# lucidrains/progen

Measured on AMD Instinct MI355X. Metric: train tokens/sec (whole node), higher is better.
Workload: dtype bf16; 1 GPU; model=ProGen-1.2B, global_batch=64, seq_len=1024, parallelism=dp1

## Files before the change

### progen_amd/ops/hip/attention_bwd.hip

```cpp

#include "common.h"

#define DH 64
#define KT 64
#define ATTN_WAVES 4
#define ATTN_BLOCK (ATTN_WAVES * WAVE)
#define NEG_INF (-1e30f)

__device__ __forceinline__ int swz(int row, int byte_in_row) {
  return (byte_in_row ^ ((row & 7) << 4));
}

__device__ __forceinline__ void load_rope(const float* rsin,
                                          const float* rcos, long long pos,
                                          int d0, float* sv, float* cv) {
  *(f32x4*)(sv) = *(const f32x4*)(rsin + pos * DH + d0);
  *(f32x4*)(sv + 4) = *(const f32x4*)(rsin + pos * DH + d0 + 4);
  *(f32x4*)(cv) = *(const f32x4*)(rcos + pos * DH + d0);
  *(f32x4*)(cv + 4) = *(const f32x4*)(rcos + pos * DH + d0 + 4);
}

__device__ __forceinline__ int uk4(int k) { return ((k & 2) >> 1) | ((k & 8) >> 2); }

typedef __attribute__((__vector_size__(4 * sizeof(__bf16)))) __bf16 bf16x4t;
#define AS3 __attribute__((address_space(3)))

#define V5_WAVES 8
#define V5_BLOCK (V5_WAVES * WAVE)

__global__ __launch_bounds__(V5_BLOCK) void attn_bwd_kernel(
    const short* __restrict__ dout, const short* __restrict__ qkv,
    const short* __restrict__ halo,
    const short* __restrict__ out, const float* __restrict__ lse,
    float* __restrict__ dacc, float* __restrict__ dlook,
    float* __restrict__ dhalo,
    int B, int N, int H, int wsz) {
  const int window = blockIdx.x;
  const int head = blockIdx.y;
  const int batch = blockIdx.z;

  const int lane = threadIdx.x % WAVE;
  const int wid = threadIdx.x / WAVE;
  const int l15 = lane & 15;
  const int l4 = lane >> 4;
  const int pid = wid >> 1;
  const int phalf = wid & 1;

  const long long HD3 = 3LL * H * DH;
  const long long HD = (long long)H * DH;
  const long long HD2 = 2LL * H * DH;
  const long long qkv_bn = (long long)batch * N * HD3;
  const long long o_bn = (long long)batch * N * HD;
  const int q_off = head * DH;
  const int k_off = H * DH + head * DH;
  const int v_off = 2 * H * DH + head * DH;
  const long long look_bn = (long long)batch * N * HD2;
  const int lk_off = head * DH;
  const int lv_off = H * DH + head * DH;

  extern __shared__ __attribute__((aligned(16))) char smem[];
  char* k_lds = smem;
  char* kt_lds = smem + 8192;
  char* v_lds = smem + 16384;
  char* qt_base = smem + 24576;
  char* dot_base = qt_base + 4 * 8192;
  char* pds_base = dot_base + 4 * 8192;
  char* ds2_base = pds_base + 4 * 8192;
  float* d_base = (float*)(ds2_base + 4 * 8192);
  float* lse_base = (float*)(ds2_base + 4 * 8192 + 1024);

  char* qt_lds = qt_base + pid * 8192;
  char* dot_lds = dot_base + pid * 8192;
  char* pds_lds = pds_base + pid * 8192;
  char* ds2_lds = ds2_base + pid * 8192;
  float* d_lds = d_base + pid * 64;
  float* lse_lds = lse_base + pid * 64;

  const float scale = rsqrtf((float)DH);
  const int tiles = 2 * wsz / KT;
  const int chunks64 = wsz / 64;
  const int rounds = (chunks64 + 3) / 4;

  const int su_key = (int)threadIdx.x >> 3;
  const int su_d0 = ((int)threadIdx.x & 7) * 8;

  for (int round = 0; round < rounds; ++round) {
    const int c64 = round * 4 + pid;
    const bool active = c64 < chunks64;
    const int nactive = min(4, chunks64 - round * 4);
    const int chunk_off = c64 * 64 + phalf * 32;
    const int q0 = window * wsz + chunk_off;
    const int colbase = phalf * 32;

    bf16x8 qfrag[2][2];
    f32x4 dqacc[2][4];
#pragma unroll
    for (int m = 0; m < 2; ++m)
#pragma unroll
      for (int d = 0; d < 4; ++d) dqacc[m][d] = (f32x4){0.f, 0.f, 0.f, 0.f};

    if (active) {
#pragma unroll
      for (int m = 0; m < 2; ++m) {
        const int row = q0 + m * 16 + l15;
#pragma unroll
        for (int ks = 0; ks < 2; ++ks) {
          const int d0 = ks * 32 + 8 * l4;
          bf16x8 v = *(const bf16x8*)(qkv + qkv_bn + (long long)row * HD3 +
                                      q_off + d0);
          bf16x8 o;
#pragma unroll
          for (int j = 0; j < 8; ++j)
            ((short*)&o)[j] = f2bf(bf2f(((short*)&v)[j]) * scale);
          qfrag[m][ks] = o;
        }
      }
      {
        const int row = lane >> 1;
        const int col = colbase + row;
        const long long gq = qkv_bn + (long long)(q0 + row) * HD3 + q_off;
        const long long go = o_bn + (long long)(q0 + row) * HD + head * DH;
        float dsum = 0.f;
#pragma unroll
        for (int gg = 0; gg < 4; ++gg) {
          const int g = (lane & 1) * 4 + gg;
          const int d0 = g * 8;
          bf16x8 qv = *(const bf16x8*)(qkv + gq + d0);
          bf16x8 ov = *(const bf16x8*)(out + go + d0);
          bf16x8 dov = *(const bf16x8*)(dout + go + d0);
#pragma unroll
          for (int j = 0; j < 8; ++j) {
            const int d = d0 + j;
            *(short*)(qt_lds + d * 128 + swz(d, col * 2)) =
                f2bf(bf2f(((short*)&qv)[j]) * scale);
            *(short*)(dot_lds + d * 128 + swz(d, col * 2)) = ((short*)&dov)[j];
            dsum += bf2f(((short*)&ov)[j]) * bf2f(((short*)&dov)[j]);
          }
        }
        dsum += __shfl_xor(dsum, 1, 64);
        if ((lane & 1) == 0) {
          d_lds[col] = dsum;
          lse_lds[col] = lse[((long long)batch * H + head) * N + q0 + row];
        }
      }
    }
    __syncthreads();

    const int max_tile = active ? ((chunk_off + 31 + wsz) / KT) : -1;

    bf16x8 kreg, vreg;
    auto issue_loads = [&](int t) {
      const int kpos = (window - 1) * wsz + t * KT + su_key;
      if (kpos >= 0) {
        const long long base = qkv_bn + (long long)kpos * HD3;
        kreg = *(const bf16x8*)(qkv + base + k_off + su_d0);
        vreg = *(const bf16x8*)(qkv + base + v_off + su_d0);
      } else if (halo != nullptr) {
        const long long hb =
            ((long long)batch * wsz + (kpos + wsz)) * (2LL * H * DH);
        kreg = *(const bf16x8*)(halo + hb + head * DH + su_d0);
        vreg = *(const bf16x8*)(halo + hb + (long long)H * DH + head * DH +
                                su_d0);
      } else {
#pragma unroll
        for (int j = 0; j < 8; ++j) {
          ((short*)&kreg)[j] = 0;
          ((short*)&vreg)[j] = 0;
        }
      }
    };
    auto write_lds = [&]() {
      *(bf16x8*)(k_lds + su_key * 128 + swz(su_key, su_d0 * 2)) = kreg;
      *(bf16x8*)(v_lds + su_key * 128 + swz(su_key, su_d0 * 2)) = vreg;
#pragma unroll
      for (int j = 0; j < 8; ++j) {
        const int d = su_d0 + j;
        *(short*)(kt_lds + d * 128 + swz(d, su_key * 2)) =
            f2bf(bf2f(((short*)&kreg)[j]) * scale);
      }
    };

    issue_loads(0);
    write_lds();
    __syncthreads();

    for (int t = 0; t < tiles; ++t) {
      if (t + 1 < tiles) issue_loads(t + 1);
      const int kb = t * KT;
      const int c_min = max(0, (t * KT - wsz) / 64 - round * 4);
      const bool i_compute = active && t <= max_tile;

      if (i_compute) {
        f32x4 s[2][4];
#pragma unroll
        for (int m = 0; m < 2; ++m)
#pragma unroll
          for (int n = 0; n < 4; ++n) s[m][n] = (f32x4){0.f, 0.f, 0.f, 0.f};
        __builtin_amdgcn_s_setprio(1);
#pragma unroll
        for (int ks = 0; ks < 2; ++ks)
#pragma unroll
          for (int n = 0; n < 4; ++n) {
            const int key = n * 16 + l15;
            bf16x8 kf = *(const bf16x8*)(k_lds + key * 128 +
                                         swz(key, (ks * 32 + 8 * l4) * 2));
#pragma unroll
            for (int m = 0; m < 2; ++m)
              s[m][n] = __builtin_amdgcn_mfma_f32_16x16x32_bf16(
                  qfrag[m][ks], kf, s[m][n], 0, 0, 0);
          }
        __builtin_amdgcn_s_setprio(0);

#pragma unroll
        for (int m = 0; m < 2; ++m)
#pragma unroll
          for (int r = 0; r < 4; ++r) {
            const int rowiw = chunk_off + m * 16 + l4 * 4 + r;
            const float l = lse_lds[colbase + m * 16 + l4 * 4 + r];
#pragma unroll
            for (int n = 0; n < 4; ++n) {
              const int kpos_band = kb + n * 16 + l15;
              float v = ((float*)&s[m][n])[r];
              v = (kpos_band > rowiw + wsz) ? 0.f : __expf(v - l);
              ((float*)&s[m][n])[r] = v;
            }
          }
#pragma unroll
        for (int m = 0; m < 2; ++m)
#pragma unroll
          for (int n = 0; n < 4; ++n) {
            const int key = n * 16 + l15;
            const int row0 = colbase + m * 16 + l4 * 4;
            short pk[4];
#pragma unroll
            for (int r = 0; r < 4; ++r) pk[r] = f2bf(((float*)&s[m][n])[r]);
            *(unsigned long long*)(pds_lds + key * 128 + swz(key, row0 * 2)) =
                *(unsigned long long*)pk;
          }

        f32x4 dp[2][4];
#pragma unroll
        for (int m = 0; m < 2; ++m)
#pragma unroll
          for (int n = 0; n < 4; ++n) dp[m][n] = (f32x4){0.f, 0.f, 0.f, 0.f};
        __builtin_amdgcn_s_setprio(1);
#pragma unroll
        for (int ks = 0; ks < 2; ++ks)
#pragma unroll
          for (int m = 0; m < 2; ++m) {
            const int row = q0 + m * 16 + l15;
            const int d0 = ks * 32 + 8 * l4;
            bf16x8 dof = *(const bf16x8*)(dout + o_bn + (long long)row * HD +
                                          head * DH + d0);
#pragma unroll
            for (int n = 0; n < 4; ++n) {
              const int key = n * 16 + l15;
              bf16x8 vf = *(const bf16x8*)(v_lds + key * 128 + swz(key, d0 * 2));
              dp[m][n] = __builtin_amdgcn_mfma_f32_16x16x32_bf16(
                  dof, vf, dp[m][n], 0, 0, 0);
            }
          }
        __builtin_amdgcn_s_setprio(0);
#pragma unroll
        for (int m = 0; m < 2; ++m)
#pragma unroll
          for (int r = 0; r < 4; ++r) {
            const float dval = d_lds[colbase + m * 16 + l4 * 4 + r];
#pragma unroll
            for (int n = 0; n < 4; ++n) {
              float p = ((float*)&s[m][n])[r];
              float d = ((float*)&dp[m][n])[r];
              ((float*)&dp[m][n])[r] = p * (d - dval);
            }
          }
#pragma unroll
        for (int m = 0; m < 2; ++m)
#pragma unroll
          for (int n = 0; n < 4; ++n) {
            const int key = n * 16 + l15;
            const int row0 = colbase + m * 16 + l4 * 4;
            short dk4[4];
#pragma unroll
            for (int r = 0; r < 4; ++r) dk4[r] = f2bf(((float*)&dp[m][n])[r]);
            *(unsigned long long*)(ds2_lds + key * 128 +
                                   ((row0 * 2) ^ (uk4(key) * 32))) =
                *(unsigned long long*)dk4;
          }

        __builtin_amdgcn_s_setprio(1);
#pragma unroll
        for (int ks = 0; ks < 2; ++ks)
#pragma unroll
          for (int m = 0; m < 2; ++m) {
            const int krow1 = ks * 32 + l4 * 8 + (l15 >> 2);
            const int krow2 = krow1 + 4;
            const int colb = (colbase + m * 16 + (l15 & 3) * 4) * 2;
            auto p1 = (AS3 bf16x4t*)(ds2_lds + krow1 * 128 +
                                     (colb ^ (uk4(krow1) * 32)));
            auto p2 = (AS3 bf16x4t*)(ds2_lds + krow2 * 128 +
                                     (colb ^ (uk4(krow2) * 32)));
            bf16x4t f1 = __builtin_amdgcn_ds_read_tr16_b64_v4bf16(p1);
            bf16x4t f2 = __builtin_amdgcn_ds_read_tr16_b64_v4bf16(p2);
            bf16x8 dsf;
#pragma unroll
            for (int j = 0; j < 4; ++j) {
              ((__bf16*)&dsf)[j] = f1[j];
              ((__bf16*)&dsf)[j + 4] = f2[j];
            }
#pragma unroll
            for (int n = 0; n < 4; ++n) {
              const int d = n * 16 + l15;
              bf16x8 kf = *(const bf16x8*)(kt_lds + d * 128 +
                                           swz(d, (ks * 32 + 8 * l4) * 2));
              dqacc[m][n] = __builtin_amdgcn_mfma_f32_16x16x32_bf16(
                  dsf, kf, dqacc[m][n], 0, 0, 0);
            }
          }
        __builtin_amdgcn_s_setprio(0);
      }
      __syncthreads();

      if (t + 1 < tiles) write_lds();

      {
        const int dh0 = (wid >> 2) * 2;
        const int keyslot = (wid & 3) * 16 + l15;
        f32x4 dv[2], dk[2];
#pragma unroll
        for (int n = 0; n < 2; ++n) {
          dv[n] = (f32x4){0.f, 0.f, 0.f, 0.f};
          dk[n] = (f32x4){0.f, 0.f, 0.f, 0.f};
        }
        __builtin_amdgcn_s_setprio(1);
        for (int c = c_min; c < nactive; ++c) {
          char* pds_c = pds_base + c * 8192;
          char* ds2_c = ds2_base + c * 8192;
          char* dot_c = dot_base + c * 8192;
          char* qt_c = qt_base + c * 8192;
#pragma unroll
          for (int ks = 0; ks < 2; ++ks) {
            const int r0 = ks * 32 + 8 * l4;
            bf16x8 pf = *(const bf16x8*)(pds_c + keyslot * 128 +
                                         swz(keyslot, r0 * 2));
            bf16x8 dsf = *(const bf16x8*)(ds2_c + keyslot * 128 +
                                          ((r0 * 2) ^ (uk4(keyslot) * 32)));
#pragma unroll
            for (int n = 0; n < 2; ++n) {
              const int d = (dh0 + n) * 16 + l15;
              bf16x8 dof = *(const bf16x8*)(dot_c + d * 128 + swz(d, r0 * 2));
              bf16x8 qf = *(const bf16x8*)(qt_c + d * 128 + swz(d, r0 * 2));
              dv[n] = __builtin_amdgcn_mfma_f32_16x16x32_bf16(pf, dof, dv[n],
                                                              0, 0, 0);
              dk[n] = __builtin_amdgcn_mfma_f32_16x16x32_bf16(dsf, qf, dk[n],
                                                              0, 0, 0);
            }
          }
        }
        __builtin_amdgcn_s_setprio(0);
        const bool lookback = kb < wsz;
#pragma unroll
        for (int r = 0; r < 4; ++r) {
          const int kpos = (window - 1) * wsz + kb + (wid & 3) * 16 + l4 * 4 + r;
          float* dstv;
          float* dstk;
          if (kpos >= 0) {
            dstv = lookback
                ? dlook + look_bn + (long long)kpos * HD2 + lv_off
                : dacc + qkv_bn + (long long)kpos * HD3 + v_off;
            dstk = lookback
                ? dlook + look_bn + (long long)kpos * HD2 + lk_off
                : dacc + qkv_bn + (long long)kpos * HD3 + k_off;
          } else if (dhalo != nullptr) {
            const long long hb =
                ((long long)batch * wsz + (kpos + wsz)) * HD2;
            dstv = dhalo + hb + lv_off;
            dstk = dhalo + hb + lk_off;
          } else {
            continue;
          }
#pragma unroll
          for (int n = 0; n < 2; ++n) {
            const int dcol = (dh0 + n) * 16 + l15;
            float vv = ((float*)&dv[n])[r];
            float vk = ((float*)&dk[n])[r];
            if (round > 0) {
              vv += dstv[dcol];
              vk += dstk[dcol];
            }
            dstv[dcol] = vv;
            dstk[dcol] = vk;
          }
        }
      }
      __syncthreads();
    }

    if (active) {
#pragma unroll
      for (int m = 0; m < 2; ++m)
#pragma unroll
        for (int r = 0; r < 4; ++r) {
          const int row = q0 + m * 16 + l4 * 4 + r;
#pragma unroll
          for (int n = 0; n < 4; ++n)
            dacc[qkv_bn + (long long)row * HD3 + q_off + n * 16 + l15] =
                ((float*)&dqacc[m][n])[r];
        }
    }
    __syncthreads();
  }
}


__global__ __launch_bounds__(256) void attn_bwd_finalize_kernel(
    const float* __restrict__ dacc, const float* __restrict__ dlook,
    const float* __restrict__ rsin, const float* __restrict__ rcos,
    short* __restrict__ dqkv, int B, int N, int H, int wsz) {
  const long long HD3 = 3LL * H * DH;
  const long long HD2 = 2LL * H * DH;
  const int u = blockIdx.x * 256 + (int)threadIdx.x;
  if (u >= 3 * H * (DH / 8)) return;
  const int hslot = u >> 3;
  const int g = u & 7;
  const int d0 = g * 8;
  const long long BN = (long long)B * N;
  for (long long bn = blockIdx.y; bn < BN; bn += gridDim.y) {
    const int n = (int)(bn % N);

    const long long off = bn * HD3 + (long long)hslot * DH + d0;
    float x[8], sv[8], cv[8];
#pragma unroll
    for (int j = 0; j < 8; ++j) x[j] = dacc[off + j];
    if (hslot >= H && (n / wsz) < (N / wsz) - 1) {
      const long long loff = bn * HD2 + (long long)(hslot - H) * DH + d0;
#pragma unroll
      for (int j = 0; j < 8; ++j) x[j] += dlook[loff + j];
    }
    load_rope(rsin, rcos, n, d0, sv, cv);
#pragma unroll
    for (int p = 0; p < 4; ++p) {
      float y0 = x[2 * p], y1 = x[2 * p + 1];
      float s = sv[2 * p], c = cv[2 * p];
      x[2 * p] = y0 * c + y1 * s;
      x[2 * p + 1] = y1 * c - y0 * s;
    }
    bf16x8 o;
#pragma unroll
    for (int j = 0; j < 8; ++j) ((short*)&o)[j] = f2bf(x[j]);
    *(bf16x8*)(dqkv + off) = o;
  }
}

extern "C" {

hipError_t attn_bwd_launch(const void* dout, const void* qkv, const void* halo,
                           const float* rsin, const float* rcos,
                           const void* out, const float* lse, float* dacc,
                           float* dlook, float* dhalo, void* dqkv, int B, int N,
                           int H, int wsz, hipStream_t stream) {
  dim3 grid(N / wsz, H, B), block(V5_BLOCK);
  size_t lds = 24576 + 131072 + 2048;
  attn_bwd_kernel<<<grid, block, lds, stream>>>(
      (const short*)dout, (const short*)qkv, (const short*)halo,
      (const short*)out, lse, dacc, dlook, dhalo, B, N, H, wsz);
  hipError_t err = hipGetLastError();
  if (err != hipSuccess) return err;
  int gx = (3 * H * (DH / 8) + 255) / 256;
  long long bn_tot = (long long)B * N;
  int gy = (int)(bn_tot < 2048 ? bn_tot : 2048);
  dim3 fin_grid(gx, gy);
  attn_bwd_finalize_kernel<<<fin_grid, 256, 0, stream>>>(
      dacc, dlook, rsin, rcos, (short*)dqkv, B, N, H, wsz);
  return hipGetLastError();
}

}
```

### progen_amd/ops/hip/bindings.cpp

```cpp

#include <torch/extension.h>

#include "checks.h"
#include "kernels.h"

using namespace chk;


static std::vector<at::Tensor> ln_shift_fwd_impl(const char* op,
                                                 const at::Tensor& x,
                                                 const at::Tensor* res,
                                                 const at::Tensor& g,
                                                 bool shift, double eps) {
  const bool bf = dtype_bf16_or_fp32(op, ARG(x));
  dtype_same(op, ARG(g), ARG(x));
  if (res) dtype_same(op, Arg{"res", *res}, ARG(x));
  contiguous_rank(op, ARG(x), 3);
  const int64_t B = x.size(0), N = x.size(1), D = x.size(2);
  if (res) contiguous_shape(op, Arg{"res", *res}, x.sizes());
  contiguous_numel(op, ARG(g), D);
  multiple_of(op, "D", D, 16);
  const int Di = extent_int(op, "D", D), Ni = extent_int(op, "N", N);
  const int R = extent_int(op, "B*N", B * N);
  same_gpu(op, {ARG(x), ARG(g)});
// ... 34 lines not shown
  dtype_same(op, ARG(dy), xa);
  dtype_same(op, ARG(g), xa);
  if (ds) dtype_same(op, Arg{"ds", *ds}, xa);
  dtype_is(op, ARG(mean), at::kFloat);
  dtype_is(op, ARG(rstd), at::kFloat);
  contiguous_rank(op, xa, 3);
  const int64_t B = x.size(0), N = x.size(1), D = x.size(2);
  contiguous_shape(op, ARG(dy), x.sizes());
  if (ds) contiguous_shape(op, Arg{"ds", *ds}, x.sizes());
  contiguous_numel(op, ARG(g), D);
  contiguous_numel(op, ARG(mean), B * N);
  contiguous_numel(op, ARG(rstd), B * N);
  multiple_of(op, "D", D, 16);
  const int Di = extent_int(op, "D", D), Ni = extent_int(op, "N", N);
  const int R = extent_int(op, "B*N", B * N);
  same_gpu(op, {xa, ARG(dy), ARG(g), ARG(mean), ARG(rstd)});
  if (ds) same_gpu(op, {xa, Arg{"ds", *ds}});

  DeviceScope dev(x);
  const int nblocks = std::min(R, 1024);
  auto dx = at::empty_like(x);
  auto dw_part = at::empty({nblocks, D}, x.options().dtype(at::kFloat));
  LAUNCH(op, ln_shift_bwd_launch(
                 dy.data_ptr(), ds ? ds->data_ptr() : nullptr, x.data_ptr(),
                 g.data_ptr(), mean.data_ptr<float>(), rstd.data_ptr<float>(),
                 dx.data_ptr(), dw_part.data_ptr<float>(), nblocks, R, Ni, Di,
                 shift, bf, dev.stream));
  auto dw = dw_part.sum(0).to(x.scalar_type());
  return {dx, dw};
}

std::vector<at::Tensor> ln_shift_bwd(const at::Tensor& dy, const at::Tensor& x,
                                     const at::Tensor& g,
                                     const at::Tensor& mean,
                                     const at::Tensor& rstd, bool shift) {
  return ln_shift_bwd_impl("ln_shift_bwd", dy, c10::nullopt, ARG(x), g, mean,
                           rstd, shift);
}

std::vector<at::Tensor> ln_shift_res_bwd(const at::Tensor& dy,
                                         const c10::optional<at::Tensor>& ds,
                                         const at::Tensor& s_in,
                                         const at::Tensor& g,
                                         const at::Tensor& mean,
                                         const at::Tensor& rstd, bool shift) {
  return ln_shift_bwd_impl("ln_shift_res_bwd", dy, ds, ARG(s_in), g, mean,
                           rstd, shift);
}


at::Tensor glu_fwd(const at::Tensor& h) {
  const char* op = "glu_fwd";
  const bool bf = dtype_bf16_or_fp32(op, ARG(h));
  CHK(h.dim() >= 1, op, "h", h.dim(), "must have at least 1 dim");
  contiguous(op, ARG(h));
  const int64_t H2 = h.size(-1), rows = leading_rows(h);
  multiple_of(op, "H2", H2, 16);
  const int H = extent_int(op, "H2", H2) / 2;
  extent(op, "rows", rows, INT64_MAX);
  same_gpu(op, {ARG(h)});

  DeviceScope dev(h);
  auto sizes = h.sizes().vec();
  sizes.back() = H;
  auto y = at::empty(sizes, h.options());
  LAUNCH(op, glu_fwd_launch(h.data_ptr(), y.data_ptr(), rows, H, bf,
                            dev.stream));
  return y;
}

at::Tensor glu_bwd(const at::Tensor& dy, const at::Tensor& h) {
  const char* op = "glu_bwd";
  const bool bf = dtype_bf16_or_fp32(op, ARG(h));
  dtype_same(op, ARG(dy), ARG(h));
  CHK(h.dim() >= 1, op, "h", h.dim(), "must have at least 1 dim");
  contiguous(op, ARG(h));
  const int64_t H2 = h.size(-1), rows = leading_rows(h);
  auto dy_sizes = h.sizes().vec();
  dy_sizes.back() = H2 / 2;
  contiguous_shape(op, ARG(dy), dy_sizes);
  multiple_of(op, "H2", H2, 16);
  const int H = extent_int(op, "H2", H2) / 2;
  extent(op, "rows", rows, INT64_MAX);
  same_gpu(op, {ARG(h), ARG(dy)});

  DeviceScope dev(h);
  auto dh = at::empty_like(h);
  LAUNCH(op, glu_bwd_launch(dy.data_ptr(), h.data_ptr(), dh.data_ptr(), rows,
                            H, bf, dev.stream));
  return dh;
}

at::Tensor gelu_fwd(const at::Tensor& h) {
  const char* op = "gelu_fwd";
  const bool bf = dtype_bf16_or_fp32(op, ARG(h));
  contiguous(op, ARG(h));
  multiple_of(op, "h.numel()", h.numel(), 8);
  extent(op, "h.numel()", h.numel(), INT64_MAX);
  same_gpu(op, {ARG(h)});

  DeviceScope dev(h);
  auto y = at::empty_like(h);
  LAUNCH(op, gelu_fwd_launch(h.data_ptr(), y.data_ptr(), h.numel(), bf,
                             dev.stream));
  return y;
}

at::Tensor gelu_bwd(const at::Tensor& dy, const at::Tensor& h) {
  const char* op = "gelu_bwd";
  const bool bf = dtype_bf16_or_fp32(op, ARG(h));
  dtype_same(op, ARG(dy), ARG(h));
  contiguous(op, ARG(h));
  contiguous_shape(op, ARG(dy), h.sizes());
  multiple_of(op, "h.numel()", h.numel(), 8);
  extent(op, "h.numel()", h.numel(), INT64_MAX);
  same_gpu(op, {ARG(h), ARG(dy)});

  DeviceScope dev(h);
  auto dh = at::empty_like(h);
  LAUNCH(op, gelu_bwd_launch(dy.data_ptr(), h.data_ptr(), dh.data_ptr(),
                             h.numel(), bf, dev.stream));
  return dh;
}


static constexpr int64_t kCeMaxRows = 4 * (int64_t)INT_MAX;

std::vector<at::Tensor> ce_fwd(const at::Tensor& logits,
                               const at::Tensor& targets) {
  const char* op = "ce_fwd";
  const bool bf = dtype_bf16_or_fp32(op, ARG(logits));
  dtype_is(op, ARG(targets), at::kLong);
  CHK(logits.dim() >= 1, op, "logits", logits.dim(),
      "must have at least 1 dim");
  contiguous(op, ARG(logits));
  const int64_t R = leading_rows(logits);
  contiguous_numel(op, ARG(targets), R);
  const int V = extent_int(op, "V", logits.size(-1));
  extent(op, "rows", R, kCeMaxRows);
  same_gpu(op, {ARG(logits), ARG(targets)});

  DeviceScope dev(logits);
  auto nll = at::empty(targets.sizes(), logits.options().dtype(at::kFloat));
  auto lse = at::empty_like(nll);
  LAUNCH(op, ce_fwd_launch(logits.data_ptr(),
                           (const long long*)targets.data_ptr<int64_t>(),
                           nll.data_ptr<float>(), lse.data_ptr<float>(), R, V,
                           bf, dev.stream));
  return {nll, lse};
}

at::Tensor ce_bwd(const at::Tensor& dnll, const at::Tensor& logits,
                  const at::Tensor& targets, const at::Tensor& lse) {
  const char* op = "ce_bwd";
  const bool bf = dtype_bf16_or_fp32(op, ARG(logits));
  dtype_is(op, ARG(targets), at::kLong);
  dtype_is(op, ARG(dnll), at::kFloat);
  dtype_is(op, ARG(lse), at::kFloat);
  CHK(logits.dim() >= 1, op, "logits", logits.dim(),
      "must have at least 1 dim");
  contiguous(op, ARG(logits));
  const int64_t R = leading_rows(logits);
  contiguous_numel(op, ARG(targets), R);
  contiguous_numel(op, ARG(dnll), R);
  contiguous_numel(op, ARG(lse), R);
  const int V = extent_int(op, "V", logits.size(-1));
  extent(op, "rows", R, kCeMaxRows);
  same_gpu(op, {ARG(logits), ARG(targets), ARG(dnll), ARG(lse)});

  DeviceScope dev(logits);
  auto dlogits = at::empty_like(logits);
  LAUNCH(op, ce_bwd_launch(dnll.data_ptr<float>(), logits.data_ptr(),
                           (const long long*)targets.data_ptr<int64_t>(),
                           lse.data_ptr<float>(), dlogits.data_ptr(), R, V, bf,
                           dev.stream));
  return dlogits;
}


at::Tensor grad_sumsq(const at::Tensor& grads) {
  const char* op = "grad_sumsq";
  const bool bf = dtype_bf16_or_fp32(op, ARG(grads));
  contiguous(op, ARG(grads));
  multiple_of(op, "grads.numel()", grads.numel(), bf ? 8 : 4);
  extent(op, "grads.numel()", grads.numel(), INT64_MAX);
  same_gpu(op, {ARG(grads)});

  DeviceScope dev(grads);
  auto out = at::zeros({1}, grads.options().dtype(at::kFloat));
  LAUNCH(op, grad_sumsq_launch(grads.data_ptr(), out.data_ptr<float>(),
                               grads.numel(), bf, dev.stream));
  return out;
}

void fused_adamw(at::Tensor& master, at::Tensor& params,
                 const at::Tensor& grads, at::Tensor& exp_avg,
                 at::Tensor& exp_avg_sq, const at::Tensor& chunk_starts,
                 const at::Tensor& chunk_ends, const at::Tensor& chunk_decay,
                 double lr, double b1, double b2, double eps, double wd,
                 at::Tensor& step_dev, double grad_scale,
                 const at::Tensor& clip_coef, int64_t shard_off) {
  const char* op = "fused_adamw";
  const bool bf = dtype_bf16_or_fp32(op, ARG(params));
  dtype_same(op, ARG(grads), ARG(params));
  dtype_is(op, ARG(master), at::kFloat);
  dtype_is(op, ARG(exp_avg), at::kFloat);
  dtype_is(op, ARG(exp_avg_sq), at::kFloat);
  dtype_is(op, ARG(chunk_starts), at::kLong);
  dtype_is(op, ARG(chunk_ends), at::kLong);
  dtype_is(op, ARG(chunk_decay), at::kInt);
  dtype_is(op, ARG(step_dev), at::kInt);
  dtype_is(op, ARG(clip_coef), at::kFloat);
  contiguous(op, ARG(params));
  contiguous(op, ARG(master));
  contiguous(op, ARG(chunk_starts));
  contiguous_numel(op, ARG(grads), params.numel());
  contiguous_numel(op, ARG(exp_avg), master.numel());
  contiguous_numel(op, ARG(exp_avg_sq), master.numel());
  contiguous_numel(op, ARG(chunk_ends), chunk_starts.numel());
  contiguous_numel(op, ARG(chunk_decay), chunk_starts.numel());
  contiguous_numel(op, ARG(step_dev), 1);
  contiguous_numel(op, ARG(clip_coef), 1);
  CHK(shard_off >= 0, op, "shard_off", shard_off, "must be >= 0");
  CHK(shard_off <= params.numel() - master.numel(), op,
      "shard_off + master.numel()", shard_off + master.numel(),
      "must be <= params.numel() = ", params.numel());
  const int nchunks = extent_int(op, "nchunks", chunk_starts.numel());
  same_gpu(op, {ARG(params), ARG(grads), ARG(master), ARG(exp_avg),
                ARG(exp_avg_sq), ARG(chunk_starts), ARG(chunk_ends),
                ARG(chunk_decay), ARG(step_dev), ARG(clip_coef)});

  DeviceScope dev(params);
  LAUNCH(op, fused_adamw_launch(
                 master.data_ptr<float>(), params.data_ptr(), grads.data_ptr(),
                 exp_avg.data_ptr<float>(), exp_avg_sq.data_ptr<float>(),
                 (const long long*)chunk_starts.data_ptr<int64_t>(),
                 (const long long*)chunk_ends.data_ptr<int64_t>(),
                 chunk_decay.data_ptr<int>(), nchunks, (float)lr, (float)b1,
                 (float)b2, (float)eps, (float)wd, step_dev.data_ptr<int>(),
                 (float)grad_scale, clip_coef.data_ptr<float>(), bf,
                 (long long)shard_off, dev.stream));
}


at::Tensor rope_qkv(const at::Tensor& qkv, const at::Tensor& rsin,
                    const at::Tensor& rcos) {
  const char* op = "rope_qkv";
  dtype_is(op, ARG(qkv), at::kBFloat16);
  dtype_is(op, ARG(rsin), at::kFloat);
  dtype_is(op, ARG(rcos), at::kFloat);
  contiguous_rank(op, ARG(qkv), 3);
  const int64_t B = qkv.size(0), N = qkv.size(1), C = qkv.size(2);
  rope_table(op, ARG(rsin), N);
  rope_table(op, ARG(rcos), N);
  multiple_of(op, "qkv.size(2)", C, 3 * 64);
  const int Bi = extent_int(op, "B", B), Ni = extent_int(op, "N", N);
  const int H = extent_int(op, "heads", C / (3 * 64));
  same_gpu(op, {ARG(qkv), ARG(rsin), ARG(rcos)});

  DeviceScope dev(qkv);
  auto qkv_rot = at::empty_like(qkv);
  LAUNCH(op, rope_qkv_launch(qkv.data_ptr(), rsin.data_ptr<float>(),
                             rcos.data_ptr<float>(), qkv_rot.data_ptr(), Bi,
                             Ni, H, dev.stream));
  return qkv_rot;
}

std::vector<at::Tensor> attn_fwd(const at::Tensor& qkv_rot, int64_t heads,
                                 int64_t window,
                                 const c10::optional<at::Tensor>& halo) {
  const char* op = "attn_fwd";
  const int H = extent_int(op, "heads", heads, kGridYZ);
  const int wsz = extent_int(op, "window", window);
  dtype_is(op, ARG(qkv_rot), at::kBFloat16);
  if (halo) dtype_same(op, Arg{"halo", *halo}, ARG(qkv_rot));
  contiguous_rank(op, ARG(qkv_rot), 3);
  const int64_t B = qkv_rot.size(0), N = qkv_rot.size(1);
  CHK(qkv_rot.size(2) == 3 * heads * 64, op, "qkv_rot.size(2)",
      qkv_rot.size(2), "must be 3*heads*64 = ", 3 * heads * 64);
  if (halo)
    contiguous_shape(op, Arg{"halo", *halo}, {B, window, 2 * heads * 64});
  multiple_of(op, "window", window, 64);
  multiple_of(op, "N", N, window);
  const int Bi = extent_int(op, "B", B, kGridYZ);
  const int Ni = extent_int(op, "N", N);
  same_gpu(op, {ARG(qkv_rot)});
  if (halo) same_gpu(op, {ARG(qkv_rot), Arg{"halo", *halo}});

  DeviceScope dev(qkv_rot);
  auto out = at::empty({B, N, heads * 64}, qkv_rot.options());
  auto lse = at::empty({B, heads, N}, qkv_rot.options().dtype(at::kFloat));
  LAUNCH(op, attn_fwd_launch(qkv_rot.data_ptr(),
                             halo ? halo->data_ptr() : nullptr, out.data_ptr(),
                             lse.data_ptr<float>(), Bi, Ni, H, wsz,
                             dev.stream));
  return {out, lse};
}

std::vector<at::Tensor> attn_bwd(const at::Tensor& dout, const at::Tensor& qkv,
                                 const at::Tensor& rsin,
                                 const at::Tensor& rcos, const at::Tensor& out,
                                 const at::Tensor& lse, int64_t heads,
                                 int64_t window,
                                 const c10::optional<at::Tensor>& halo) {
  const char* op = "attn_bwd";
  const int H = extent_int(op, "heads", heads, kGridYZ);
  const int wsz = extent_int(op, "window", window);
  dtype_is(op, ARG(qkv), at::kBFloat16);
  dtype_same(op, ARG(dout), ARG(qkv));
  dtype_same(op, ARG(out), ARG(qkv));
  if (halo) dtype_same(op, Arg{"halo", *halo}, ARG(qkv));
  dtype_is(op, ARG(lse), at::kFloat);
  dtype_is(op, ARG(rsin), at::kFloat);
  dtype_is(op, ARG(rcos), at::kFloat);
  contiguous_rank(op, ARG(qkv), 3);
  const int64_t B = qkv.size(0), N = qkv.size(1);
  CHK(qkv.size(2) == 3 * heads * 64, op, "qkv.size(2)", qkv.size(2),
      "must be 3*heads*64 = ", 3 * heads * 64);
  contiguous_shape(op, ARG(out), {B, N, heads * 64});
  contiguous_shape(op, ARG(dout), {B, N, heads * 64});
  contiguous_shape(op, ARG(lse), {B, heads, N});
  rope_table(op, ARG(rsin), N);
  rope_table(op, ARG(rcos), N);
  if (halo)
    contiguous_shape(op, Arg{"halo", *halo}, {B, window, 2 * heads * 64});
  multiple_of(op, "window", window, 64);
  multiple_of(op, "N", N, window);
  const int Bi = extent_int(op, "B", B, kGridYZ);
  const int Ni = extent_int(op, "N", N);
  same_gpu(op, {ARG(qkv), ARG(dout), ARG(out), ARG(lse), ARG(rsin),
                ARG(rcos)});
  if (halo) same_gpu(op, {ARG(qkv), Arg{"halo", *halo}});

  DeviceScope dev(qkv);
  const auto f32 = qkv.options().dtype(at::kFloat);
  auto dacc = at::empty_like(qkv, f32);
  auto dlook = at::empty({B, N, 2 * heads * 64}, f32);
  auto dqkv = at::empty_like(qkv);
  auto dhalo = halo ? at::empty({B, window, 2 * heads * 64}, f32)
                    : at::Tensor();
  LAUNCH(op, attn_bwd_launch(
                 dout.data_ptr(), qkv.data_ptr(),
                 halo ? halo->data_ptr() : nullptr, rsin.data_ptr<float>(),
                 rcos.data_ptr<float>(), out.data_ptr(), lse.data_ptr<float>(),
                 dacc.data_ptr<float>(), dlook.data_ptr<float>(),
                 halo ? dhalo.data_ptr<float>() : nullptr, dqkv.data_ptr(), Bi,
                 Ni, H, wsz, dev.stream));
  if (halo) return {dqkv, dhalo};
  return {dqkv};
}


std::vector<at::Tensor> sgu_fwd(const at::Tensor& xa, const at::Tensor& g_ln,
                                const at::Tensor& w, const at::Tensor& bias) {
  const char* op = "sgu_fwd";
  dtype_is(op, ARG(xa), at::kBFloat16);
  dtype_same(op, ARG(g_ln), ARG(xa));
  dtype_same(op, ARG(w), ARG(xa));
  contiguous_rank(op, ARG(xa), 3);
  const int64_t B = xa.size(0), N = xa.size(1), D = xa.size(2);
  contiguous_shape(op, ARG(g_ln), xa.sizes());
  contiguous_shape(op, ARG(w), {N, N});
  CHK(bias.numel() == N, op, "bias", bias.numel(), "must have ", N,
      " elements");
  multiple_of(op, "N", N, 256);
  multiple_of(op, "D", D, 64);
  const int Bi = extent_int(op, "B", B, kGridYZ);
  const int Ni = extent_int(op, "N", N);
  const int Di = extent_int(op, "D", D, 64 * kGridYZ);
  same_gpu(op, {ARG(xa), ARG(g_ln), ARG(w), ARG(bias)});

  DeviceScope dev(xa);
  auto bias_f = bias.to(at::kFloat).contiguous().view({-1});
  auto out = at::empty_like(xa);
  auto gate_out = at::empty_like(xa);
  LAUNCH(op, sgu_fwd_launch(xa.data_ptr(), g_ln.data_ptr(), w.data_ptr(),
                            bias_f.data_ptr<float>(), out.data_ptr(),
                            gate_out.data_ptr(), Bi, Ni, Di, dev.stream));
  return {out, gate_out};
}

at::Tensor sgu_dgate(const at::Tensor& t_in, const at::Tensor& w) {
  const char* op = "sgu_dgate";
  dtype_is(op, ARG(t_in), at::kBFloat16);
  dtype_same(op, ARG(w), ARG(t_in));
  contiguous_rank(op, ARG(t_in), 3);
  const int64_t B = t_in.size(0), N = t_in.size(1), D = t_in.size(2);
  contiguous_shape(op, ARG(w), {N, N});
  multiple_of(op, "N", N, 256);
  multiple_of(op, "D", D, 64);
  const int Bi = extent_int(op, "B", B, kGridYZ);
  const int Ni = extent_int(op, "N", N);
  const int Di = extent_int(op, "D", D, 64 * kGridYZ);
  same_gpu(op, {ARG(t_in), ARG(w)});

  DeviceScope dev(t_in);
  auto dg = at::empty_like(t_in);
  LAUNCH(op, sgu_dgate_launch(t_in.data_ptr(), w.data_ptr(), dg.data_ptr(),
                              Bi, Ni, Di, dev.stream));
  return dg;
}

at::Tensor sgu_dw(const at::Tensor& t_in, const at::Tensor& g_ln,
                  const at::Tensor& tri_m, const at::Tensor& tri_k) {
  const char* op = "sgu_dw";
  dtype_is(op, ARG(t_in), at::kBFloat16);
  dtype_same(op, ARG(g_ln), ARG(t_in));
  dtype_is(op, ARG(tri_m), at::kInt);
  dtype_is(op, ARG(tri_k), at::kInt);
  contiguous_rank(op, ARG(t_in), 3);
  const int64_t B = t_in.size(0), N = t_in.size(1), D = t_in.size(2);
  contiguous_shape(op, ARG(g_ln), t_in.sizes());
  contiguous(op, ARG(tri_m));
  contiguous_numel(op, ARG(tri_k), tri_m.numel());
  multiple_of(op, "N", N, 64);
  multiple_of(op, "D", D, 32);
  const int ntri = extent_int(op, "tri_m.numel()", tri_m.numel());
  const int Bi = extent_int(op, "B", B, kGridYZ);
  const int Ni = extent_int(op, "N", N);
  const int Di = extent_int(op, "D", D, 768 * kGridYZ);
  same_gpu(op, {ARG(t_in), ARG(g_ln), ARG(tri_m), ARG(tri_k)});

  DeviceScope dev(t_in);
  auto dw = at::zeros({N, N}, t_in.options().dtype(at::kFloat));
  LAUNCH(op, sgu_dw_launch(t_in.data_ptr(), g_ln.data_ptr(),
                           dw.data_ptr<float>(), tri_m.data_ptr<int>(),
                           tri_k.data_ptr<int>(), ntri, Bi, Ni, Di,
                           dev.stream));
  return dw;
}


static const uint32_t* crc32c_tables() {
  static uint32_t tbl[8][256];
  static bool init = false;
  if (!init) {
    for (int i = 0; i < 256; ++i) {
      uint32_t c = (uint32_t)i;
      for (int k = 0; k < 8; ++k) c = (c >> 1) ^ ((c & 1) ? 0x82F63B78u : 0);
      tbl[0][i] = c;
    }
    for (int t = 1; t < 8; ++t)
      for (int i = 0; i < 256; ++i)
        tbl[t][i] = (tbl[t - 1][i] >> 8) ^ tbl[0][tbl[t - 1][i] & 0xFF];
    init = true;
  }
  return &tbl[0][0];
}

uint32_t crc32c_host(py::bytes data) {
  const uint32_t* T = crc32c_tables();
  char* buf;
  Py_ssize_t len;
  if (PyBytes_AsStringAndSize(data.ptr(), &buf, &len) != 0)
    throw std::runtime_error("crc32c: expected bytes");
  const uint8_t* p = (const uint8_t*)buf;
  uint32_t c = 0xFFFFFFFFu;
  size_t n = (size_t)len;
  while (n >= 8) {
    uint32_t lo, hi;
    memcpy(&lo, p, 4);
    memcpy(&hi, p + 4, 4);
    lo ^= c;
    c = T[7 * 256 + (lo & 0xFF)] ^ T[6 * 256 + ((lo >> 8) & 0xFF)] ^
        T[5 * 256 + ((lo >> 16) & 0xFF)] ^ T[4 * 256 + (lo >> 24)] ^
        T[3 * 256 + (hi & 0xFF)] ^ T[2 * 256 + ((hi >> 8) & 0xFF)] ^
        T[1 * 256 + ((hi >> 16) & 0xFF)] ^ T[0 * 256 + (hi >> 24)];
    p += 8;
    n -= 8;
  }
  while (n--) c = T[(c ^ *p++) & 0xFF] ^ (c >> 8);
  return c ^ 0xFFFFFFFFu;
}

at::Tensor colsum(const at::Tensor& dy) {
  const char* op = "colsum";
  dtype_is(op, ARG(dy), at::kBFloat16);
  contiguous_rank(op, ARG(dy), 2);
  multiple_of(op, "C", dy.size(1), 8);
  extent(op, "R", dy.size(0), INT_MAX);
  const int C = extent_int(op, "C", dy.size(1));
  same_gpu(op, {ARG(dy)});

  DeviceScope dev(dy);
  auto out = at::zeros({dy.size(1)}, dy.options().dtype(at::kFloat));
  LAUNCH(op, colsum_launch(dy.data_ptr(), out.data_ptr<float>(), dy.size(0),
                           C, dev.stream));
  return out;
}

at::Tensor fp8_quantize(const at::Tensor& t, const at::Tensor& scale) {
  const char* op = "fp8_quantize";
  dtype_is(op, ARG(t), at::kBFloat16);
  dtype_is(op, ARG(scale), at::kFloat);
  contiguous(op, ARG(t));
  contiguous_numel(op, ARG(scale), 1);
  multiple_of(op, "t.numel()", t.numel(), 8);
  extent(op, "t.numel()", t.numel(), INT64_MAX);
  same_gpu(op, {ARG(t), ARG(scale)});

  DeviceScope dev(t);
  auto out = at::empty_like(t, t.options().dtype(at::kFloat8_e4m3fn));
  LAUNCH(op, quant_e4m3_launch(t.data_ptr(), out.data_ptr(),
                               scale.data_ptr<float>(), t.numel(),
                               dev.stream));
  return out;
}

at::Tensor fp8_quantize_t(const at::Tensor& w, const at::Tensor& scale) {
  const char* op = "fp8_quantize_t";
  dtype_is(op, ARG(w), at::kBFloat16);
  dtype_is(op, ARG(scale), at::kFloat);
  contiguous_rank(op, ARG(w), 2);
  contiguous_numel(op, ARG(scale), 1);
  multiple_of(op, "rows", w.size(0), 2);
  const int Nr = extent_int(op, "rows", w.size(0));
  const int Kc = extent_int(op, "cols", w.size(1));
  extent(op, "tiles", ((w.size(0) + 63) / 64) * ((w.size(1) + 63) / 64),
         INT_MAX);
  same_gpu(op, {ARG(w), ARG(scale)});

  DeviceScope dev(w);
  auto out = at::empty({w.size(1), w.size(0)},
                       w.options().dtype(at::kFloat8_e4m3fn));
  LAUNCH(op, quant_e4m3_t_launch(w.data_ptr(), out.data_ptr(),
                                 scale.data_ptr<float>(), Nr, Kc, dev.stream));
  return out;
}

PYBIND11_MODULE(TORCH_EXTENSION_NAME, m) {
  m.def("sgu_fwd", &sgu_fwd, "SGU causal spatial matmul forward");
  m.def("sgu_dgate", &sgu_dgate, "SGU backward: dgate");
  m.def("sgu_dw", &sgu_dw, "SGU backward: dW");
  m.def("ln_shift_fwd", &ln_shift_fwd, "fused LN+shift forward");
  m.def("ln_shift_bwd", &ln_shift_bwd, "fused LN+shift backward");
  m.def("ln_shift_res_fwd", &ln_shift_res_fwd,
        "residual-add-fused LN+shift forward");
  m.def("ln_shift_res_bwd", &ln_shift_res_bwd,
        "residual-add-fused LN+shift backward");
  m.def("glu_fwd", &glu_fwd, "GLU-GELU forward");
  m.def("glu_bwd", &glu_bwd, "GLU-GELU backward");
  m.def("gelu_fwd", &gelu_fwd, "GELU forward");
  m.def("gelu_bwd", &gelu_bwd, "GELU backward");
  m.def("ce_fwd", &ce_fwd, "fused CE forward (nll, lse)");
  m.def("ce_bwd", &ce_bwd, "fused CE backward");
  m.def("grad_sumsq", &grad_sumsq, "sum of squares of flat grads");
  m.def("fused_adamw", &fused_adamw, "fused clip+AdamW over flat space",
        py::arg("master"), py::arg("params"), py::arg("grads"),
        py::arg("exp_avg"), py::arg("exp_avg_sq"), py::arg("chunk_starts"),
        py::arg("chunk_ends"), py::arg("chunk_decay"), py::arg("lr"),
        py::arg("b1"), py::arg("b2"), py::arg("eps"), py::arg("wd"),
        py::arg("step_dev"), py::arg("grad_scale"), py::arg("clip_coef"),
        py::arg("shard_off") = 0);
  m.def("rope_qkv", &rope_qkv, "pre-rotation of qkv (rotary on q,k,v)");
  m.def("attn_fwd", &attn_fwd, "fused local attention forward",
        py::arg("qkv_rot"), py::arg("heads"), py::arg("window"),
        py::arg("halo") = py::none());
  m.def("attn_bwd", &attn_bwd, "fused local attention backward",
        py::arg("dout"), py::arg("qkv"), py::arg("rsin"), py::arg("rcos"),
        py::arg("out"), py::arg("lse"), py::arg("heads"), py::arg("window"),
        py::arg("halo") = py::none());
  m.def("crc32c", &crc32c_host, "CRC-32C (slicing-by-8, host)");
  m.def("colsum", &colsum, "bf16 column sum (bias grads), fp32 accum");
  m.def("fp8_quantize", &fp8_quantize, "fused bf16 -> e4m3 at device scale");
  m.def("fp8_quantize_t", &fp8_quantize_t,
        "fused transpose-quantize (N,K) bf16 -> (K,N) e4m3");
}
```

### progen_amd/ops/hip/kernels.h

```cpp
#pragma once
#include <hip/hip_runtime.h>

extern "C" {

hipError_t ln_shift_fwd_launch(const void* x, const void* res, const void* g,
                               void* y, void* s_out, float* mean, float* rstd,
                               int R, int N, int D, float eps, bool shift,
                               bool is_bf16, hipStream_t stream);
hipError_t ln_shift_bwd_launch(const void* dy, const void* ds, const void* x,
                               const void* g, const float* mean,
                               const float* rstd, void* dx, float* dw_part,
                               int nblocks, int R, int N, int D, bool shift,
                               bool is_bf16, hipStream_t stream);

hipError_t glu_fwd_launch(const void* h, void* y, long long rows, int H,
                          bool is_bf16, hipStream_t stream);
hipError_t glu_bwd_launch(const void* dy, const void* h, void* dh,
                          long long rows, int H, bool is_bf16,
                          hipStream_t stream);
hipError_t gelu_fwd_launch(const void* h, void* y, long long total_elems,
                           bool is_bf16, hipStream_t stream);
hipError_t gelu_bwd_launch(const void* dy, const void* h, void* dh,
                           long long total_elems, bool is_bf16,
                           hipStream_t stream);

hipError_t ce_fwd_launch(const void* logits, const long long* targets,
                         float* nll, float* lse, long long R, int V,
                         bool is_bf16, hipStream_t stream);
hipError_t ce_bwd_launch(const float* dnll, const void* logits,
                         const long long* targets, const float* lse,
                         void* dlogits, long long R, int V, bool is_bf16,
                         hipStream_t stream);

hipError_t grad_sumsq_launch(const void* grads, float* out, long long numel,
                             bool is_bf16, hipStream_t stream);
hipError_t fused_adamw_launch(float* master, void* params, const void* grads,
                              float* exp_avg, float* exp_avg_sq,
                              const long long* starts, const long long* ends,
                              const int* decay_flags, int nchunks, float lr,
                              float b1, float b2, float eps, float wd,
                              int* step_dev, float grad_scale,
                              const float* clip_coef, bool is_bf16,
                              long long shard_off, hipStream_t stream);

hipError_t colsum_launch(const void* dy, float* out, long long R, int C,
                         hipStream_t stream);
hipError_t quant_e4m3_launch(const void* in, void* out, const float* scale,
                             long long numel, hipStream_t stream);
hipError_t quant_e4m3_t_launch(const void* in, void* out, const float* scale,
                               int Nr, int Kc, hipStream_t stream);

hipError_t rope_qkv_launch(const void* qkv, const float* rsin,
                           const float* rcos, void* qkv_rot, int B, int N,
                           int H, hipStream_t stream);
hipError_t attn_fwd_launch(const void* qkv_rot, const void* halo, void* out,
                           float* lse, int B, int N, int H, int wsz,
                           hipStream_t stream);
hipError_t attn_bwd_launch(const void* dout, const void* qkv, const void* halo,
                           const float* rsin, const float* rcos,
                           const void* out, const float* lse, float* dacc,
                           float* dlook, float* dhalo, void* dqkv, int B, int N,
                           int H, int wsz, hipStream_t stream);

hipError_t sgu_fwd_launch(const void* xa, const void* g_ln, const void* w,
                          const float* bias, void* out, void* gate_out, int B,
                          int N, int D, hipStream_t stream);
hipError_t sgu_dgate_launch(const void* t_in, const void* w, void* dg, int B,
                            int N, int D, hipStream_t stream);
hipError_t sgu_dw_launch(const void* t_in, const void* g_ln, float* dw,
                         const int* tri_m, const int* tri_k, int ntri, int B,
                         int N, int D, hipStream_t stream);

}
```

Before: 100,400 tokens/s.

## Fuse attention backward windows into one kernel with in-kernel inverse-rope epilogue

Adds a fused variant of the local-attention backward kernel. Each block loops over all windows of a (head, batch) pair, carries lookback dK/dV partials in a small fp32 carry buffer, and applies the inverse rotary transform directly when writing bf16 dQKV. This removes the full fp32 dacc/dlook scratch tensors and the second rope/accumulate kernel. In exchange the grid shrinks to B*H blocks with windows processed serially, so it is only picked when B*H is large. It also writes packed bf16 pairs using lane shuffles.

```diff
diff --git a/progen_amd/ops/hip/attention_bwd.hip b/progen_amd/ops/hip/attention_bwd.hip
--- a/progen_amd/ops/hip/attention_bwd.hip
+++ b/progen_amd/ops/hip/attention_bwd.hip
@@ -28,19 +28,42 @@
 #define V5_WAVES 8
 #define V5_BLOCK (V5_WAVES * WAVE)
 
+__device__ __forceinline__ short inv_rot_bf16(float self, float partner,
+                                              float c, float s_signed) {
+  return f2bf(__fmaf_rn(self, c, __fmul_rn(partner, s_signed)));
+}
+
+#ifndef ATTN_BWD_PACKED_STORE
+#define ATTN_BWD_PACKED_STORE 1
+#endif
+#if ATTN_BWD_PACKED_STORE
+constexpr int kEpiR = 2;
+__device__ __forceinline__ int epi_r(int e, int l15) { return e + 2 * (l15 & 1); }
+#else
+constexpr int kEpiR = 4;
+__device__ __forceinline__ int epi_r(int e, int) { return e; }
+#endif
+
+template <bool FUSED>
 __global__ __launch_bounds__(V5_BLOCK) void attn_bwd_kernel(
     const short* __restrict__ dout, const short* __restrict__ qkv,
     const short* __restrict__ halo,
     const short* __restrict__ out, const float* __restrict__ lse,
     float* __restrict__ dacc, float* __restrict__ dlook,
     float* __restrict__ dhalo,
-    int B, int N, int H, int wsz) {
-  const int window = blockIdx.x;
+    const float* __restrict__ rsin, const float* __restrict__ rcos,
+    float* carry,
+    short* __restrict__ dqkv, int B, int N, int H, int wsz) {
+  const int nwin = N / wsz;
+  const int w_begin = FUSED ? 0 : (int)blockIdx.x;
+  const int w_end = FUSED ? nwin : w_begin + 1;
   const int head = blockIdx.y;
   const int batch = blockIdx.z;
 
-  const int lane = threadIdx.x % WAVE;
-  const int wid = threadIdx.x / WAVE;
+  for (int window = w_begin; window < w_end; ++window) {
+  const int tid = threadIdx.x;
+  const int lane = tid % WAVE;
+  const int wid = tid / WAVE;
   const int l15 = lane & 15;
   const int l4 = lane >> 4;
   const int pid = wid >> 1;
@@ -81,8 +104,8 @@
   const int chunks64 = wsz / 64;
   const int rounds = (chunks64 + 3) / 4;
 
-  const int su_key = (int)threadIdx.x >> 3;
-  const int su_d0 = ((int)threadIdx.x & 7) * 8;
+  const int su_key = tid >> 3;
+  const int su_d0 = (tid & 7) * 8;
 
   for (int round = 0; round < rounds; ++round) {
     const int c64 = round * 4 + pid;
@@ -100,6 +123,15 @@
       for (int d = 0; d < 4; ++d) dqacc[m][d] = (f32x4){0.f, 0.f, 0.f, 0.f};
 
     if (active) {
+      int ptid = tid;
+      if constexpr (FUSED) asm volatile("" : "+v"(ptid));
+      const int lane = ptid % WAVE, l15 = lane & 15, l4 = lane >> 4;
+      const int ppid = ptid / WAVE >> 1, colbase = (ptid / WAVE & 1) * 32;
+      const int q0 = window * wsz + (round * 4 + ppid) * 64 + colbase;
+      char* qt_lds = qt_base + ppid * 8192;
+      char* dot_lds = dot_base + ppid * 8192;
+      float* d_lds = d_base + ppid * 64;
+      float* lse_lds = lse_base + ppid * 64;
 #pragma unroll
       for (int m = 0; m < 2; ++m) {
         const int row = q0 + m * 16 + l15;
@@ -331,6 +363,40 @@
           dv[n] = (f32x4){0.f, 0.f, 0.f, 0.f};
           dk[n] = (f32x4){0.f, 0.f, 0.f, 0.f};
         }
+        const bool lookback = kb < wsz;
+        const bool fin = FUSED && (lookback ? window > 0 : window == nwin - 1);
+        const bool add = FUSED && lookback && window > 0;
+        const int kt0 = (window - 1) * wsz + kb;
+        const int keyq = (wid & 3) * 16 + l4 * 4;
+        const int dcol0 = dh0 * 16 + l15;
+        f32x4* cbase = nullptr;
+        f32x4 cin[2][2];
+        float esin[2][kEpiR], ecos[2][kEpiR];
+        if constexpr (FUSED) {
+          const int ctile = lookback ? t : t - chunks64;
+          cbase = (f32x4*)carry +
+                  (((long long)batch * H + head) * chunks64 + ctile) * 2048;
+          if (add) {
+#pragma unroll
+            for (int n = 0; n < 2; ++n)
+#pragma unroll
+              for (int kv = 0; kv < 2; ++kv)
+                cin[n][kv] = cbase[(n * 2 + kv) * 512 + tid];
+          }
+          if (fin) {
+            const float* ts = rsin + (long long)kt0 * DH;
+            const float* tc = rcos + (long long)kt0 * DH;
+#pragma unroll
+            for (int n = 0; n < 2; ++n)
+#pragma unroll
+              for (int e = 0; e < kEpiR; ++e) {
+                const int ti = (keyq + epi_r(e, l15)) * DH +
+                               ((dcol0 + n * 16) & ~1);
+                esin[n][e] = ts[ti];
+                ecos[n][e] = tc[ti];
+              }
+          }
+        }
         __builtin_amdgcn_s_setprio(1);
         for (int c = c_min; c < nactive; ++c) {
           char* pds_c = pds_base + c * 8192;
@@ -357,7 +423,58 @@
           }
         }
         __builtin_amdgcn_s_setprio(0);
-        const bool lookback = kb < wsz;
+        if (fin) {
+#pragma unroll
+          for (int n = 0; n < 2; ++n) {
+            if (add) {
+#pragma unroll
+              for (int r = 0; r < 4; ++r) {
+                ((float*)&dk[n])[r] =
+                    __fadd_rn(((float*)&cin[n][0])[r], ((float*)&dk[n])[r]);
+                ((float*)&dv[n])[r] =
+                    __fadd_rn(((float*)&cin[n][1])[r], ((float*)&dv[n])[r]);
+              }
+            }
+            const bool odd = l15 & 1;
+            const int hd3 = 3 * H * DH;
+#pragma unroll
+            for (int kv = 0; kv < 2; ++kv) {
+              const float* y = kv ? (const float*)&dv[n] : (const float*)&dk[n];
+              short* dst = dqkv + qkv_bn + (long long)kt0 * HD3 +
+                           (kv ? v_off : k_off);
+              const int col = dcol0 + n * 16;
+#if ATTN_BWD_PACKED_STORE
+#pragma unroll
+              for (int e = 0; e < 2; ++e) {
+                const float a = y[e], b = y[e + 2];
+                const float recv = __shfl_xor(odd ? a : b, 1, 64);
+                const float y0 = odd ? recv : a;
+                const float y1 = odd ? b : recv;
+                const unsigned lo = (unsigned short)inv_rot_bf16(
+                    y0, y1, ecos[n][e], esin[n][e]);
+                const unsigned hi = (unsigned short)inv_rot_bf16(
+                    y1, y0, ecos[n][e], -esin[n][e]);
+                *(unsigned*)(dst + (keyq + epi_r(e, l15)) * hd3 + (col & ~1)) =
+                    lo | (hi << 16);
+              }
+#else
+#pragma unroll
+              for (int r = 0; r < 4; ++r) {
+                const float other = __shfl_xor(y[r], 1, 64);
+                dst[(keyq + r) * hd3 + col] =
+                    inv_rot_bf16(y[r], other, ecos[n][r],
+                                 odd ? -esin[n][r] : esin[n][r]);
+              }
+#endif
+            }
+          }
+        } else if (FUSED && !lookback) {
+#pragma unroll
+          for (int n = 0; n < 2; ++n) {
+            cbase[(n * 2 + 0) * 512 + tid] = dk[n];
+            cbase[(n * 2 + 1) * 512 + tid] = dv[n];
+          }
+        } else {
 #pragma unroll
         for (int r = 0; r < 4; ++r) {
           const int kpos = (window - 1) * wsz + kb + (wid & 3) * 16 + l4 * 4 + r;
@@ -391,11 +508,53 @@
             dstk[dcol] = vk;
           }
         }
+        }
       }
       __syncthreads();
     }
 
-    if (active) {
+    if (FUSED && active) {
+      int etid = threadIdx.x;
+      asm volatile("" : "+v"(etid));
+      const int elane = etid % WAVE, ewid = etid / WAVE;
+      const int el15 = elane & 15, el4 = elane >> 4;
+      char* bounce = ((ewid & 1) ? dot_base : qt_base) + (ewid >> 1) * 8192;
+      const int eq0 = window * wsz + (ewid >> 1) * 64 + (ewid & 1) * 32;
+#pragma unroll
+      for (int m = 0; m < 2; ++m)
+#pragma unroll
+        for (int r = 0; r < 4; ++r) {
+          const int brow = m * 16 + el4 * 4 + r;
+#pragma unroll
+          for (int n = 0; n < 4; ++n)
+            *(float*)(bounce + brow * 256 +
+                      (((n * 16 + el15) * 4) ^ (el4 << 6))) =
+                ((float*)&dqacc[m][n])[r];
+        }
+      const short* dq_w = dqkv + qkv_bn + (long long)eq0 * HD3 + q_off;
+      const float* sin_w = rsin + (long long)eq0 * DH;
+      const float* cos_w = rcos + (long long)eq0 * DH;
+#pragma unroll
+      for (int i = 0; i < 4; ++i) {
+        const int brow = i * 8 + (elane >> 3);
+        const int d0 = (elane & 7) * 8;
+        const int boff = brow * 256 + ((d0 * 4) ^ (((brow >> 2) & 3) << 6));
+        float x[8], sv[8], cv[8];
+        *(f32x4*)(x) = *(const f32x4*)(bounce + boff);
+        *(f32x4*)(x + 4) = *(const f32x4*)(bounce + boff + 16);
+        load_rope(sin_w, cos_w, brow, d0, sv, cv);
+        bf16x8 o;
+#pragma unroll
+        for (int p = 0; p < 4; ++p) {
+          ((short*)&o)[2 * p] =
+              inv_rot_bf16(x[2 * p], x[2 * p + 1], cv[2 * p], sv[2 * p]);
+          ((short*)&o)[2 * p + 1] =
+              inv_rot_bf16(x[2 * p + 1], x[2 * p], cv[2 * p], -sv[2 * p]);
+        }
+        *(bf16x8*)((short*)dq_w + brow * (3 * H * DH) + d0) = o;
+      }
+    }
+    if (!FUSED && active) {
 #pragma unroll
       for (int m = 0; m < 2; ++m)
 #pragma unroll
@@ -408,6 +567,7 @@
         }
     }
     __syncthreads();
+  }
   }
 }
 
@@ -434,35 +594,54 @@
     if (hslot >= H && (n / wsz) < (N / wsz) - 1) {
       const long long loff = bn * HD2 + (long long)(hslot - H) * DH + d0;
 #pragma unroll
-      for (int j = 0; j < 8; ++j) x[j] += dlook[loff + j];
+      for (int j = 0; j < 8; ++j) x[j] = __fadd_rn(x[j], dlook[loff + j]);
     }
     load_rope(rsin, rcos, n, d0, sv, cv);
+    bf16x8 o;
 #pragma unroll
     for (int p = 0; p < 4; ++p) {
-      float y0 = x[2 * p], y1 = x[2 * p + 1];
-      float s = sv[2 * p], c = cv[2 * p];
-      x[2 * p] = y0 * c + y1 * s;
-      x[2 * p + 1] = y1 * c - y0 * s;
+      ((short*)&o)[2 * p] =
+          inv_rot_bf16(x[2 * p], x[2 * p + 1], cv[2 * p], sv[2 * p]);
+      ((short*)&o)[2 * p + 1] =
+          inv_rot_bf16(x[2 * p + 1], x[2 * p], cv[2 * p], -sv[2 * p]);
     }
-    bf16x8 o;
-#pragma unroll
-    for (int j = 0; j < 8; ++j) ((short*)&o)[j] = f2bf(x[j]);
     *(bf16x8*)(dqkv + off) = o;
   }
 }
 
+#define ATTN_BWD_FUSED_MIN_HB 1536
+
 extern "C" {
+
+int attn_bwd_fused_supported(int wsz) { return wsz <= 4 * 64; }
+
+int attn_bwd_pick_fused(int B, int N, int H, int wsz) {
+  (void)N;
+  return attn_bwd_fused_supported(wsz) &&
+         (long long)H * B >= ATTN_BWD_FUSED_MIN_HB;
+}
 
 hipError_t attn_bwd_launch(const void* dout, const void* qkv, const void* halo,
                            const float* rsin, const float* rcos,
                            const void* out, const float* lse, float* dacc,
-                           float* dlook, float* dhalo, void* dqkv, int B, int N,
-                           int H, int wsz, hipStream_t stream) {
-  dim3 grid(N / wsz, H, B), block(V5_BLOCK);
+                           float* dlook, float* dhalo, float* carry,
+                           void* dqkv, int B, int N, int H, int wsz, int fused,
+                           hipStream_t stream) {
+  dim3 block(V5_BLOCK);
   size_t lds = 24576 + 131072 + 2048;
-  attn_bwd_kernel<<<grid, block, lds, stream>>>(
+  if (fused) {
+    if (!attn_bwd_fused_supported(wsz)) return hipErrorInvalidValue;
+    attn_bwd_kernel<true><<<dim3(1, H, B), block, lds, stream>>>(
+        (const short*)dout, (const short*)qkv, (const short*)halo,
+        (const short*)out, lse, nullptr, nullptr, dhalo, rsin, rcos, carry,
+        (short*)dqkv, B, N, H, wsz);
+    return hipGetLastError();
+  }
+  dim3 grid(N / wsz, H, B);
+  attn_bwd_kernel<false><<<grid, block, lds, stream>>>(
       (const short*)dout, (const short*)qkv, (const short*)halo,
-      (const short*)out, lse, dacc, dlook, dhalo, B, N, H, wsz);
+      (const short*)out, lse, dacc, dlook, dhalo, nullptr, nullptr, nullptr,
+      nullptr, B, N, H, wsz);
   hipError_t err = hipGetLastError();
   if (err != hipSuccess) return err;
   int gx = (3 * H * (DH / 8) + 255) / 256;
diff --git a/progen_amd/ops/hip/bindings.cpp b/progen_amd/ops/hip/bindings.cpp
--- a/progen_amd/ops/hip/bindings.cpp
+++ b/progen_amd/ops/hip/bindings.cpp
@@ -360,7 +360,8 @@
                                  const at::Tensor& rcos, const at::Tensor& out,
                                  const at::Tensor& lse, int64_t heads,
                                  int64_t window,
-                                 const c10::optional<at::Tensor>& halo) {
+                                 const c10::optional<at::Tensor>& halo,
+                                 c10::optional<bool> fused) {
   const char* op = "attn_bwd";
   const int H = extent_int(op, "heads", heads, kGridYZ);
   const int wsz = extent_int(op, "window", window);
@@ -390,10 +391,20 @@
                 ARG(rcos)});
   if (halo) same_gpu(op, {ARG(qkv), Arg{"halo", *halo}});
 
+  CHK(!(fused && *fused) || attn_bwd_fused_supported(wsz), op, "fused=True",
+      window, "must have window <= 256 (a single round of chunks)");
+  const bool use_fused =
+      fused ? *fused : attn_bwd_pick_fused(Bi, Ni, H, wsz) != 0;
+
   DeviceScope dev(qkv);
   const auto f32 = qkv.options().dtype(at::kFloat);
-  auto dacc = at::empty_like(qkv, f32);
-  auto dlook = at::empty({B, N, 2 * heads * 64}, f32);
+  at::Tensor dacc, dlook, carry;
+  if (use_fused) {
+    carry = at::empty({B * heads * window * 128}, f32);
+  } else {
+    dacc = at::empty_like(qkv, f32);
+    dlook = at::empty({B, N, 2 * heads * 64}, f32);
+  }
   auto dqkv = at::empty_like(qkv);
   auto dhalo = halo ? at::empty({B, window, 2 * heads * 64}, f32)
                     : at::Tensor();
@@ -401,11 +412,24 @@
                  dout.data_ptr(), qkv.data_ptr(),
                  halo ? halo->data_ptr() : nullptr, rsin.data_ptr<float>(),
                  rcos.data_ptr<float>(), out.data_ptr(), lse.data_ptr<float>(),
-                 dacc.data_ptr<float>(), dlook.data_ptr<float>(),
-                 halo ? dhalo.data_ptr<float>() : nullptr, dqkv.data_ptr(), Bi,
-                 Ni, H, wsz, dev.stream));
+                 use_fused ? nullptr : dacc.data_ptr<float>(),
+                 use_fused ? nullptr : dlook.data_ptr<float>(),
+                 halo ? dhalo.data_ptr<float>() : nullptr,
+                 use_fused ? carry.data_ptr<float>() : nullptr,
+                 dqkv.data_ptr(), Bi, Ni, H, wsz, use_fused ? 1 : 0,
+                 dev.stream));
   if (halo) return {dqkv, dhalo};
   return {dqkv};
+}
+
+std::string attn_bwd_path(int64_t B, int64_t N, int64_t heads,
+                          int64_t window) {
+  const char* op = "_attn_bwd_path";
+  const int H = extent_int(op, "heads", heads, kGridYZ);
+  const int wsz = extent_int(op, "window", window);
+  const int Bi = extent_int(op, "B", B, kGridYZ);
+  const int Ni = extent_int(op, "N", N);
+  return attn_bwd_pick_fused(Bi, Ni, H, wsz) ? "fused" : "two_kernel";
 }
 
 
@@ -617,7 +641,10 @@
   m.def("attn_bwd", &attn_bwd, "fused local attention backward",
         py::arg("dout"), py::arg("qkv"), py::arg("rsin"), py::arg("rcos"),
         py::arg("out"), py::arg("lse"), py::arg("heads"), py::arg("window"),
-        py::arg("halo") = py::none());
+        py::arg("halo") = py::none(), py::arg("fused") = py::none());
+  m.def("_attn_bwd_path", &attn_bwd_path,
+        "path attn_bwd picks when fused is None: 'fused' or 'two_kernel'",
+        py::arg("B"), py::arg("N"), py::arg("heads"), py::arg("window"));
   m.def("crc32c", &crc32c_host, "CRC-32C (slicing-by-8, host)");
   m.def("colsum", &colsum, "bf16 column sum (bias grads), fp32 accum");
   m.def("fp8_quantize", &fp8_quantize, "fused bf16 -> e4m3 at device scale");
diff --git a/progen_amd/ops/hip/kernels.h b/progen_amd/ops/hip/kernels.h
--- a/progen_amd/ops/hip/kernels.h
+++ b/progen_amd/ops/hip/kernels.h
@@ -59,8 +59,11 @@
 hipError_t attn_bwd_launch(const void* dout, const void* qkv, const void* halo,
                            const float* rsin, const float* rcos,
                            const void* out, const float* lse, float* dacc,
-                           float* dlook, float* dhalo, void* dqkv, int B, int N,
-                           int H, int wsz, hipStream_t stream);
+                           float* dlook, float* dhalo, float* carry,
+                           void* dqkv, int B, int N, int H, int wsz, int fused,
+                           hipStream_t stream);
+int attn_bwd_fused_supported(int wsz);
+int attn_bwd_pick_fused(int B, int N, int H, int wsz);
 
 hipError_t sgu_fwd_launch(const void* xa, const void* g_ln, const void* w,
                           const float* bias, void* out, void* gate_out, int B,
```

Measured after the change: 103,400 tokens/s, median of 6. 1.03x the previous value.
